# theo2021/OnDA

Hardware: AMD Instinct MI355X
Metric: adaptation-step images/sec (fwd+bwd+proto) 512x1024 bs=4 (higher is better)
Workload: dtype f32 (f16x2 split emulation); 1 GPU; hybrid_switch adaptation step (step + update_ema), 1024x512, bs=4 per micro-batch, 1 micro-batch(es) per GPU and optimizer step, dynamic branch, DeepLabV2-ResNet50 ProDA head, random-init weights; global_batch=4, parallelism=dp1, branch=dynamic, micro_batches_per_gpu=1, inputs=resident in HBM

## Files before the change

include/onda_hip.h:

```cpp
#ifndef ONDA_HIP_H
#define ONDA_HIP_H

#include <stdint.h>

#ifdef __cplusplus
extern "C" {
#endif

typedef void* onda_stream_t;

#define ONDA_OK 0
#define ONDA_EINVAL (-1)
#define ONDA_EALIGN (-2)

typedef struct OndaConv {
  int B, Hi, Wi, Cin;
  int Ho, Wo, Cout;
  int kh, kw, stride, dil, pad;
  int ldx;
  int ldy;
  int ldr;
  int out_os;
  int Hf, Wf;
  int relu;
// ... 66 lines not shown
                        float* running_mean, float* running_var, int64_t* nbt, float momentum, const float* gamma,
                        const float* beta, const float* res_amax, int relu, float* xhat_amax, float* out_amax, int64_t split,
                        int tile_rows, int run_group, const float* y, int ldy, onda_stream_t s);
int onda_bn_apply_l2(const float* x, const float* mean, const float* invstd, const float* gamma, const float* beta,
                     const void* res, int64_t res_plane, const float* res_amax, void* out, int64_t out_plane,
                     const float* out_amax, int64_t M, int C, int relu, uint8_t* relu_mask, int64_t split, onda_stream_t s);
int onda_bn_train_l2(const float* x, const float* partials, int tiles, float eps, float* mean, float* invstd, float* running_mean,
                     float* running_var, int64_t* nbt, float momentum, const float* gamma, const float* beta, const void* res,
                     const float* res_amax, int relu, float* xhat_amax, void* out, float* out_amax, int64_t M, int C,
                     uint8_t* relu_mask, int64_t split, int tile_rows, int run_group, onda_stream_t s);
int64_t onda_bn_bwd_l2_ws(int64_t M, int C);
int onda_bn_bwd_l2(const float* dout, const void* out, int64_t out_plane, const float* x, const float* mean, const float* invstd,
                   const float* gamma, const float* xhat_amax, void* dx, int64_t dx_plane, float* dx_amax, float* dres, float* ws,
                   int64_t M, int C, int relu, const uint8_t* relu_mask, int64_t split, int fuse_sums, onda_stream_t s);

int onda_conv_wgrad_l2_variant(int Cout, int Cin);
int64_t onda_conv2d_wgrad_l2_table_stride(const OndaConv* c);
int onda_conv2d_wgrad_l2_table(const OndaConv* c, int32_t* table, onda_stream_t s);
int onda_conv2d_wgrad_l2(const void* xl, int64_t xplane, const float* xamax, const void* dyl, int64_t dyplane, const float* dyamax,
                         float* slabs, int lddy, int splitk, const OndaConv* c, onda_stream_t s);

int onda_conv2d_wgrad(const float* x, const float* dy, float* slabs, int lddy, int splitk,
                      const OndaConv* c, onda_stream_t s);
int onda_wgrad_reduce(const float* slabs, float* dw, int splitk, int Cout, int taps, int Cin,
                      int Cout_real, int Cin_real, int flat_k, int accumulate, onda_stream_t s);

int onda_pack_weight_fwd(const float* w_oihw, float* dst, int Cout, int Cin, int taps, int Cout_pad, int Kp,
                         onda_stream_t s);
int onda_pack_weight_dgrad(const float* w_oihw, float* dst, int Cout, int Cin, int taps, int Cout_pad,
                           onda_stream_t s);
// ... 160 lines not shown
```

onda_amd/_lib.py:

```python
import ctypes
import os
from ctypes import POINTER, Structure, c_char_p, c_float, c_int, c_int64, c_void_p

HERE = os.path.dirname(os.path.abspath(__file__))
LIB_PATH = os.environ.get("ONDA_LIB_PATH") or os.path.join(HERE, "libonda_hip.so")

P = c_void_p
I, L, F = c_int, c_int64, c_float


class OndaConv(Structure):
    _fields_ = [(n, c_int) for n in ("B Hi Wi Cin Ho Wo Cout kh kw stride dil pad ldx ldy ldr out_os Hf Wf relu").split()] + \
               [("run_if", c_void_p), ("stat_split", c_int64), ("plain_schedule", c_int), ("pix_table", c_void_p),
                ("pix_stride", c_int64)]


class OndaSwitchCfg(Structure):
    _fields_ = [("limit", c_int), ("level_kind", c_int), ("use_exp", c_int), ("pad_", c_int), ("exp_const", ctypes.c_double),
                ("one_minus_exp_const", ctypes.c_double), ("taps_total", ctypes.c_double), ("gray_lo", ctypes.c_double),
                ("gray_hi", ctypes.c_double), ("dev_threshold", ctypes.c_double)]


class OndaLimbOut(Structure):
    _fields_ = [("out", c_void_p), ("out_plane", c_int64), ("out_bound", c_void_p), ("out_amax", c_void_p), ("kb", c_void_p),
                ("xtrue", c_void_p), ("res", c_void_p), ("res_plane", c_int64), ("res_amax", c_void_p), ("res_true", c_void_p)]


class OndaSgdEntry(Structure):
    _fields_ = [("p", c_void_p), ("g", c_void_p), ("buf", c_void_p), ("n", c_int64), ("lr", c_float),
                ("times", c_int), ("fresh", c_int), ("first_block", c_int)]


class OndaSgdAnchorEntry(Structure):
    _fields_ = [("p", c_void_p), ("g", c_void_p), ("buf", c_void_p), ("anchor", c_void_p), ("n", c_int64), ("lr", c_float),
                ("times", c_int), ("fresh", c_int), ("first_block", c_int)]


class OndaSqdiffEntry(Structure):
    _fields_ = [("a", c_void_p), ("b", c_void_p), ("n", c_int64), ("first_block", c_int)]

# ... 35 lines not shown
    "onda_conv_l2_kernel_id": (I, [L, I, I, I]),
    "onda_conv_l2_tiles_m": (I, [L, I, I, I]),
    "onda_conv_l2_tiles_m_split": (I, [L, I, I, I, L, I, POINTER(c_int)]),
    "onda_conv_l2_live_fraction": (ctypes.c_double, [POINTER(OndaConv), I]),
    "onda_conv_wgrad_l2_live_fraction": (ctypes.c_double, [POINTER(OndaConv), I]),
    "onda_conv_wgrad_l2_variant": (I, [I, I]),
    "onda_conv2d_wgrad_l2_table_stride": (L, [POINTER(OndaConv)]),
    "onda_conv2d_wgrad_l2_table": (I, [POINTER(OndaConv), P, P]),
    "onda_conv2d_wgrad_l2": (I, [P, L, P, P, L, P, P, I, I, POINTER(OndaConv), P]),
    "onda_conv2d_fwd_l2": (I, [P, L, P, P, P, P, P, P, P, P, I, P, P, POINTER(OndaConv), P]),
    "onda_bn_finalize_l2": (I, [P, I, I, L, F, P, P, P, P, P, F, P, P, P, I, P, P, L, I, I, P, I, P]),
    "onda_bn_apply_l2": (I, [P, P, P, P, P, P, L, P, P, L, P, L, I, I, P, L, P]),
    "onda_bn_bwd_l2_ws": (L, [L, I]),
    "onda_bn_train_l2": (I, [P, P, I, F, P, P, P, P, P, F, P, P, P, P, I, P, P, P, L, I, P, L, I, I, P]),
    "onda_bn_bwd_l2": (I, [P, P, L, P, P, P, P, P, P, L, P, P, P, L, I, I, P, L, I, P]),
    "onda_conv2d_wgrad": (I, [P, P, P, I, I, POINTER(OndaConv), P]),
    "onda_wgrad_reduce": (I, [P, P, I, I, I, I, I, I, I, I, P]),
    "onda_pack_weight_fwd": (I, [P, P, I, I, I, I, I, P]),
    "onda_pack_weight_dgrad": (I, [P, P, I, I, I, I, P]),
    "onda_stem_im2col": (I, [P, P, I, I, I, I, I, I, P]),
    "onda_bn_finalize": (I, [P, I, I, L, F, P, P, P, P, P, F, P]),
    "onda_bn_stats": (I, [P, L, I, I, P, POINTER(c_int), P]),
    "onda_bn_apply": (I, [P, P, P, P, P, P, P, L, I, I, P, P]),
    "onda_bn_fold": (I, [P, P, P, P, F, P, P, I, P]),
    "onda_bn_bwd_ws": (L, [L, I]),
    "onda_bn_bwd": (I, [P, P, P, P, P, P, P, P, P, L, I, I, P, P]),
    "onda_gn_ws": (L, [I, L, I]),
    "onda_gn_fwd": (I, [P, I, P, P, P, P, I, P, P, P, I, L, I, I, F, I, P, P]),
    "onda_gn_bwd": (I, [P, I, P, I, P, I, P, P, P, P, P, P, P, P, I, L, I, I, I, P]),
    "onda_gn_site_ws": (L, [I, L, I]),
# ... 90 lines not shown
```

onda_amd/csrc/norm_l2.hip:

```cpp
#include "limbs.h"

namespace {

#define LD4(p) (*reinterpret_cast<const f32x4*>(p))

__device__ __forceinline__ void store_limb_lines(_Float16* o, u32x4 l1, u32x4 l2, bool whole) {
  if (!whole) {
    *reinterpret_cast<u32x4*>(o) = l1;
    *reinterpret_cast<u32x4*>(o + LIMB2_OFS) = l2;
    return;
  }
  const bool hi = (threadIdx.x & 4) != 0;
  const u32x4 send = hi ? l1 : l2;
  u32x4 recv;
#pragma unroll
  for (int j = 0; j < 4; ++j) recv[j] = (unsigned)__shfl_xor((int)send[j], 4, 64);
  const unsigned long long mine = reinterpret_cast<unsigned long long>(o);
  const unsigned long long partner = ((unsigned long long)(unsigned)__shfl_xor((int)(mine >> 32), 4, 64) << 32) |
                                     (unsigned)__shfl_xor((int)(unsigned)mine, 4, 64);
  _Float16* po = reinterpret_cast<_Float16*>(partner);
  _Float16* a1 = hi ? po + LIMB2_OFS : o;
  _Float16* a2 = hi ? o + LIMB2_OFS : po;
  *reinterpret_cast<u32x4*>(a1) = hi ? recv : l1;
  *reinterpret_cast<u32x4*>(a2) = hi ? l2 : recv;
// ... 110 lines not shown
  const float* partials;
  int tiles, C;
  double count;
  float eps;
  float *mean, *invstd, *rmean, *rvar;
  int64_t* nbt;
  float momentum;
  const float *gamma, *beta, *res_amax;
  int relu;
  float *xhat_amax, *out_amax;
  long long split;
  int bm, run_group;
  const float* y;
  int ldy;
};
__device__ __forceinline__ void bn_finalize_block(const BnFinalizeArgs& a, const int bx, const int g) {
  const float* __restrict__ partials = a.partials;
  const int tiles = a.tiles, C = a.C, relu = a.relu, bm = a.bm, run_group = a.run_group, ldy = a.ldy;
  double count = a.count;
  const float eps = a.eps, momentum = a.momentum;
  float *mean = a.mean, *invstd = a.invstd, *rmean = a.rmean, *rvar = a.rvar, *xhat_amax = a.xhat_amax, *out_amax = a.out_amax;
  int64_t* nbt = a.nbt;
  const float* __restrict__ gamma = a.gamma;
  const float* __restrict__ beta = a.beta;
  const float* __restrict__ res_amax = a.res_amax;
  const float* __restrict__ y = a.y;
  const long long split = a.split;
  if (bx == 0 && g == 0 && threadIdx.x == 0 && nbt) *nbt += 1;
  int row0 = 0, nrows = tiles;
  if (split > 0) {
    const int ts = (int)(split / bm);
    if (g == 0) nrows = ts; else row0 = ts, nrows = tiles - ts;
    count = g == 0 ? (double)split : count - (double)split;
  }
  const long long m_all = (long long)a.count;
  const int tiles_m = bm > 1 ? (int)((m_all + bm - 1) / bm) : tiles, extra = tiles - tiles_m;
  int sub1 = 0;
  bool known = y != nullptr && bm > 1 && extra >= 0;
  if (known && extra > 0) {
    const bool d15 = extra % 15 == 0 && extra / 15 <= tiles_m, d31 = bm == 256 && extra % 31 == 0 && extra / 31 <= tiles_m;
// ... 7 lines not shown
    float mn = 3.0e38f, mx = -3.0e38f;
    if (bx * 16 + c < C)
      for (long long r = (split > last0 ? split : last0) + lane; r < m_all; r += 16) {
        const float v = y[(size_t)r * ldy + bx * 16 + c];
        mn = fminf(mn, v);
        mx = fmaxf(mx, v);
      }
    lmn[lane][c] = mn;
    lmx[lane][c] = mx;
  }
  double sum[2];
  float ext[2];
  reduce_rows16<4, 2, true>(partials + (size_t)row0 * 4 * C, nrows, C, bx * 16, sum, ext, rescan ? nrows - sub1 : nrows,
                            rescan ? tiles_m - 1 - row0 : -1);
  const int ch = bx * 16 + threadIdx.x;
  float bound = 0.f;
  if (threadIdx.x < 16 && ch < C) {
    if (rescan) {
#pragma unroll
      for (int l = 0; l < 16; ++l) {
        ext[0] = fminf(ext[0], lmn[l][threadIdx.x]);
        ext[1] = fmaxf(ext[1], lmx[l][threadIdx.x]);
      }
    }
    if (split > 0 && split % bm != 0) {
      double c1 = 0.0, c2 = 0.0;
      float mn = 3.0e38f, mx = -3.0e38f;
      for (long long r = split - split % bm; r < split; ++r) {
        const float v = y[(size_t)r * ldy + ch];
        c1 += (double)v;
        c2 += (double)v * (double)v;
// ... 4 lines not shown
        sum[0] += c1;
        sum[1] += c2;
        ext[0] = fminf(ext[0], mn);
        ext[1] = fmaxf(ext[1], mx);
      } else {
        sum[0] -= c1;
        sum[1] -= c2;
      }
    }
    const double mu = sum[0] / count;
    double var = sum[1] / count - mu * mu;
    if (var < 0.0) var = 0.0;
    const float muf = (float)mu, is = (float)(1.0 / sqrt(var + (double)eps));
    const float lo = (ext[0] - muf) * is, hi = (ext[1] - muf) * is;
    const float gm = gamma[ch], b = beta[ch];
    const float f_lo = lo * gm + b, f_hi = hi * gm + b;
    bound = relu ? fmaxf(0.f, fmaxf(f_lo, f_hi)) : fmaxf(fabsf(f_lo), fabsf(f_hi));
    mean[g * C + ch] = muf;
    invstd[g * C + ch] = is;
    xhat_amax[g * C + ch] = fmaxf(fabsf(lo), fabsf(hi));
    if (rmean && (split <= 0 || g == run_group)) {
      const double unbiased = count > 1.0 ? var * count / (count - 1.0) : var;
      rmean[ch] = (1.f - momentum) * rmean[ch] + momentum * muf;
      rvar[ch] = (1.f - momentum) * rvar[ch] + momentum * (float)unbiased;
    }
  }
  if (res_amax != nullptr) bound += amax_read(res_amax);
  bound *= 1.0000005f;
  __shared__ float red[4];
  float m = wave_max(bound);
  if ((threadIdx.x & 63) == 0) red[threadIdx.x >> 6] = m;
  __syncthreads();
  if (threadIdx.x == 0) {
    m = fmaxf(fmaxf(red[0], red[1]), fmaxf(red[2], red[3]));
    if (m > 0.f)
      atomicMax(reinterpret_cast<unsigned*>(out_amax) + ((bx + 7 * g) & (ONDA_AMAX_SLOTS - 1)) * AMAX_STRIDE, __float_as_uint(m));
  }
}
__global__ __launch_bounds__(256) void bn_finalize_l2_kernel(const BnFinalizeArgs a) { bn_finalize_block(a, blockIdx.x, blockIdx.y); }

template <bool FUSED>
__global__ __launch_bounds__(256) void bn_apply_l2_kernel(const float* __restrict__ x, const float* mean, const float* invstd,
                                                          const float* __restrict__ gamma, const float* __restrict__ beta,
                                                          const _Float16* __restrict__ res, size_t res_plane,
                                                          const float* __restrict__ res_amax, _Float16* __restrict__ out,
                                                          size_t out_plane, const float* out_amax, size_t total8, int C, int relu,
                                                          unsigned char* __restrict__ mask, size_t group1_at, const BnFinalizeArgs fin,
                                                          int nfin) {
  if constexpr (FUSED) {
    const int nb = (C + 15) / 16;
    if ((int)blockIdx.x < nfin) {
      bn_finalize_block(fin, blockIdx.x % nb, blockIdx.x / nb);
      grid_publish(fin.out_amax);
    }
// ... 49 lines not shown
      ra2 = ld_stream(reinterpret_cast<const u32x4*>(res + lofs(e) + LIMB2_OFS));
      rb1 = ld_stream(reinterpret_cast<const u32x4*>(res + lofs(f)));
      rb2 = ld_stream(reinterpret_cast<const u32x4*>(res + lofs(f) + LIMB2_OFS));
    }
    const bool whole = __ballot(1) == ~0ull;
    one(e, a0, a1, ra1, ra2, whole);
    one(f, b0, b1, rb1, rb2, whole);
  }
  if (e < total8) {
    u32x4 r1 = {}, r2 = {};
    if (res) {
      r1 = *reinterpret_cast<const u32x4*>(res + lofs(e));
      r2 = *reinterpret_cast<const u32x4*>(res + lofs(e) + LIMB2_OFS);
    }
    one(e, LD4(x + e * 8), LD4(x + e * 8 + 4), r1, r2, __ballot(1) == ~0ull);
  }
}

struct ColPlan3 {
  int cx, ry, gridx, chunks;
  int64_t rows_per_chunk;
};
static inline ColPlan3 col_plan3(int64_t M, int C) {
  ColPlan3 p;
  const int c4 = C / 4;
  p.cx = 1;
  while (p.cx < c4 && p.cx < 64) p.cx <<= 1;
  p.ry = 256 / p.cx;
  p.gridx = (c4 + p.cx - 1) / p.cx;
  int64_t target = 2048 / p.gridx;
// ... 152 lines not shown
    f32x4 v[2];
#pragma unroll
    for (int h = 0; h < 2; ++h) {
      const size_t o = e * 8 + 4 * h;
      f32x4 g = LD4S(dout + o);
      if (relu) g = relu_mask4(out, mask, o, g, C);
      const f32x4 xh = (LD4S(x + o) - (second ? mu[1][h] : mu[0][h])) * (second ? is[1][h] : is[0][h]);
      v[h] = (second ? gi[1][h] : gi[0][h]) * (g - (second ? m1[1][h] : m1[0][h]) - xh * (second ? m2[1][h] : m2[0][h]));
    }
    u32x4 l1, l2;
    split8(v[0] * sd, v[1] * sd, l1, l2);
    store_limb_lines(dx + (size_t)((unsigned)e / (unsigned)c8) * 2 * (size_t)C + limb_at(0, col, C), l1, l2, __ballot(1) == ~0ull);
  }
}

__global__ __launch_bounds__(256) void chan_scale_limbs_kernel(const float* __restrict__ x, const float* __restrict__ gate,
                                                               _Float16* __restrict__ out, size_t plane,
                                                               const float* __restrict__ amax, int64_t HW, int C, size_t total8) {
  const int c8 = C / 8;
  const float so = scale_of(amax).s;
  for (size_t e = (size_t)blockIdx.x * blockDim.x + threadIdx.x; e < total8; e += (size_t)gridDim.x * blockDim.x) {
    const int col = (int)(e % c8) * 8;
    const size_t b = (e / c8) / HW;
    const f32x4 v0 = LD4S(x + e * 8) * LD4(gate + b * C + col), v1 = LD4S(x + e * 8 + 4) * LD4(gate + b * C + col + 4);
    u32x4 l1, l2;
    split8(v0 * so, v1 * so, l1, l2);
    _Float16* o = out + (size_t)((unsigned)e / (unsigned)c8) * 2 * (size_t)C + limb_at(0, col, C);
    st_stream(reinterpret_cast<u32x4*>(o), l1);
    st_stream(reinterpret_cast<u32x4*>(o + LIMB2_OFS), l2);
  }
// ... 115 lines not shown
  if (fuse_sums) {
    const int nfin = (C + 15) / 16 * groups;
    const unsigned grid = ew_grid(total8) > (unsigned)nfin ? ew_grid(total8) : (unsigned)nfin;
    hipLaunchKernelGGL(bn_bwd_apply_l2_kernel<true>, dim3(grid), dim3(256), 0, st, dout, static_cast<const _Float16*>(out),
                       (size_t)out_plane, x, mean, invstd, gamma, sums, static_cast<_Float16*>(dx), (size_t)dx_plane, dx_amax, total8, C,
                       (float)inv_m0, relu, relu_mask, (size_t)split * C / 8, (float)inv_m1, fin, nfin);
    return ONDA_LAUNCH_RESULT();
  }
  hipLaunchKernelGGL(bn_bwd_sums_l2_kernel, dim3((C + 15) / 16, groups), dim3(256), 0, st, fin);
  hipLaunchKernelGGL(bn_bwd_apply_l2_kernel<false>, dim3(ew_grid(total8)), dim3(256), 0, st, dout, static_cast<const _Float16*>(out),
                     (size_t)out_plane, x, mean, invstd, gamma, sums, static_cast<_Float16*>(dx), (size_t)dx_plane, dx_amax, total8,
                     C, (float)inv_m0, relu, relu_mask, (size_t)split * C / 8, (float)inv_m1, BnBwdSumsArgs{}, 0);
  return ONDA_LAUNCH_RESULT();
}

}
```

onda_amd/framework/model/deeplabv2.py:

```python
import os

import torch
import torch.nn as nn

from onda_amd import ops

affine_par = True


class HipConv2d(nn.Conv2d):

    def __init__(self, *args, **kwargs):
        super().__init__(*args, **kwargs)
        self._pack = ops._PackCache()

    def geom(self):
        return self.kernel_size[0], self.stride[0], self.dilation[0], self.padding[0]

    def forward(self, x, want_stats=False, cout_pad=None):
        k, stride, dil, pad = self.geom()
        return ops.Conv2dFn.apply(x, self.weight, self.bias, self._pack, stride, dil, pad, want_stats, cout_pad)


class HipBatchNorm2d(nn.BatchNorm2d):
# ... 19 lines not shown
        return new




def conv_bn(conv, bn, x, relu, residual=None):
    k, stride, dil, pad = conv.geom()
    if isinstance(bn, nn.GroupNorm):
        if residual is not None:
            raise NotImplementedError("onda_amd: GroupNorm with a residual add is not a site of the reference's models")
        y, stats = conv(x, want_stats=True)
        return ops.GNSiteFn.apply(y, stats, bn.weight, bn.bias, relu, bn.num_groups, bn.eps)
    if bn.training:
        limbs = ops.limb_mode(conv.out_channels)
        y, stats = conv(x, want_stats=4 if limbs else True)
        running = (bn.running_mean, bn.running_var, bn.num_batches_tracked) if bn.track_running_stats else None
        if bn.momentum is None:
            raise NotImplementedError("onda_amd: cumulative-average BatchNorm (momentum=None) is not on the hot path")
        fn = ops.BNTrainLimbFn if stats.shape[1] == 4 else ops.BNTrainFn
        return fn.apply(y, stats, bn.weight, bn.bias, residual, relu, running, bn.momentum)
    scale, shift = bn.folded()
    with torch.no_grad():
        wp = conv._pack.get_fwd(conv.weight)
        limb_out = None
        if ops.limb_mode(conv.out_channels) and ops._use_l2(wp, x.shape[3]):
            w = conv.weight
            key = (w.data_ptr(), w._version, id(scale), id(shift))
            hit = getattr(bn, "_bound_cache", None)
            if hit is None or hit[0] != key:
                hit = bn._bound_cache = (key, ops.fold_bounds(w, scale, shift), scale, shift)
            limb_out = hit[1]
        y, _, _ = ops.conv_forward(x, wp, k, stride, dil, pad, conv.out_channels, scale=scale, shift=shift, residual=residual,
                                   relu=relu, limb_out=limb_out)
    return y


class Bottleneck(nn.Module):
    expansion = 4

    def __init__(self, inplanes, planes, stride=1, dilation=1, downsample=None, norm_module=HipBatchNorm2d,
                 norm_grad=False):
        super().__init__()
        self.conv1 = HipConv2d(inplanes, planes, kernel_size=1, stride=stride, bias=False)
        self.bn1 = norm_module(planes, affine=affine_par)
        self.conv2 = HipConv2d(planes, planes, kernel_size=3, stride=1, padding=dilation, bias=False,
                               dilation=dilation)
        self.bn2 = norm_module(planes, affine=affine_par)
        self.conv3 = HipConv2d(planes, planes * 4, kernel_size=1, bias=False)
        self.bn3 = norm_module(planes * 4, affine=affine_par)
        if not norm_grad:
            for bn in (self.bn1, self.bn2, self.bn3):
                for p in bn.parameters():
                    p.requires_grad = False
        self.relu = nn.ReLU(inplace=True)
        self.downsample = downsample
        self.stride = stride

    def forward(self, x):
        ops.share_grad(x)
        y = conv_bn(self.conv1, self.bn1, x, True)
        y = conv_bn(self.conv2, self.bn2, y, True)
        if self.downsample is not None:
            residual = conv_bn(self.downsample[0], self.downsample[1], x, False)
        else:
            residual = x
        return conv_bn(self.conv3, self.bn3, y, True, residual)


class SEBlock(nn.Module):
    def __init__(self, inplanes, r=16):
        super().__init__()
        self.global_pool = nn.AdaptiveAvgPool2d((1, 1))
        self.se = nn.Sequential(nn.Linear(inplanes, inplanes // r), nn.ReLU(inplace=True),
                                nn.Linear(inplanes // r, inplanes), nn.Sigmoid())

    def forward(self, x):
        return ops.SEScaleFn.apply(x, self.se[0].weight, self.se[0].bias, self.se[2].weight, self.se[2].bias)
# ... 225 lines not shown
```

onda_amd/ops/__init__.py:

```python
import sys
import types

from . import _state, conv, core, disc, limbs, loss, norm, tables
from ._state import BN_EPS, GN_EPS, GN_GROUPS, HEAD_PAD, STEM_K

_FLAGS = ("CONV_MODE", "H2_PATH", "GRAD_READY", "PROFILE", "PREDICATE", "ROW_GROUPS", "LIMB_ONLY", "SHARE_GRADS", "FUSE_BN_FINALIZE",
          "GN_FUSED_STATS")

for _m in (core, limbs, tables, conv, norm, loss, disc):
    for _k, _v in vars(_m).items():
        if not _k.startswith("__") and _k not in _FLAGS and not isinstance(_v, types.ModuleType):
            globals()[_k] = _v
del _m, _k, _v


class _OpsModule(types.ModuleType):
    def __getattr__(self, name):
        if name in _FLAGS:
            return getattr(_state, name)
        raise AttributeError(f"module {self.__name__!r} has no attribute {name!r}")

    def __setattr__(self, name, value):
        if name in _FLAGS:
            setattr(_state, name, value)
# ... 6 lines not shown
```

onda_amd/ops/_state.py:

```python
import os

BN_EPS = 1e-5
GN_EPS = 1e-5
GN_GROUPS = 32
HEAD_PAD = 32
STEM_K = 160


CONV_MODE = os.environ.get("ONDA_CONV_MODE", "f16x2")

H2_PATH = "dma"

GRAD_READY = None

PROFILE = None



PREDICATE = None

ROW_GROUPS = 0

LIMB_ONLY = True

SHARE_GRADS = True

FUSE_BN_FINALIZE = os.environ.get("ONDA_FUSE_BN", "0") == "1"

GN_FUSED_STATS = os.environ.get("ONDA_GN_FUSED_STATS", "1") == "1"
```

onda_amd/ops/norm.py:

```python
import ctypes
import os
from ctypes import byref

import torch

from .. import _lib
from .._lib import OndaConv, OndaLimbOut, call, query
from . import _state
from ._state import BN_EPS, GN_EPS, GN_GROUPS, HEAD_PAD, STEM_K
from .core import _group_split, _p, _stream, as_nhwc, nhwc_ld
from .limbs import Limbs, _stat_tile_rows, amax_slot, is_limb_only, known_amax, limb_mode, limb_only, limbs_of, tag_amax
from .conv import _sink_give, _sink_of, colsum


class BNTrainFn(torch.autograd.Function):

    @staticmethod
    def _groups(B, H, W):
        split, M = _group_split(B, H, W), B * H * W
        return [(0, M)] if not split else [(0, split), (split, M - split)]

    @staticmethod
    def forward(ctx, y, stats, gamma, beta, residual, relu, running, momentum):
        B, H, W, C = y.shape
# ... 120 lines not shown
        need_res = ctx.has_res and ctx.needs_input_grad[4]
        dres = None
        if need_res:
            dres = torch.empty_like(y) if ctx.relu else dout
        ol = ctx.out_limbs
        call("onda_bn_bwd_l2", _p(dout), _p(ol.planes) if ol is not None else None, ol.plane if ol is not None else 0, _p(y),
             _p(mean), _p(invstd), _p(gamma), _p(xhat_amax), _p(planes), M * C, _p(dx_amax),
             _p(dres) if (need_res and ctx.relu) else None, _p(ws), M, C, int(ctx.relu), _p(ctx.relu_mask), ctx.split,
             int(_state.FUSE_BN_FINALIZE), _stream())
        dx = limb_only((B, H, W, C), dev, Limbs(planes, dx_amax, C, M * C))
        if need_res:
            dres = _sink_give(ctx.res_sink, dres, ctx.relu)
        return dx, None, None, None, dres, None, None, None


def fold_bounds(weight, scale, shift):
    with torch.no_grad():
        l1 = weight.detach().abs().sum(dim=(1, 2, 3))
        return torch.stack([(scale.abs() * l1).max(), shift.abs().max()]).float().contiguous()


def bn_eval_fold(gamma, beta, rm, rv):
    C = gamma.numel()
    scale = torch.empty(C, device=gamma.device, dtype=torch.float32)
    shift = torch.empty_like(scale)
    call("onda_bn_fold", _p(gamma), _p(beta), _p(rm), _p(rv), BN_EPS, _p(scale), _p(shift), C, _stream())
    return scale, shift


class MaxPoolFn(torch.autograd.Function):
# ... 173 lines not shown
```

Before: 43.40 images/s.

## Fuse downsample and main-branch BatchNorm pairs in bottleneck blocks

Adds paired BN kernels that finalize statistics for both the conv3 BN and the downsample BN in one launch. The forward pass normalizes both, adds them, applies ReLU and writes f16 limbs in a single pass. The backward pass reads dout once to compute both branches' reductions and dx. This removes the intermediate residual limb tensor and its separate write and read, and cuts kernel launches in the four downsample bottlenecks. In exchange it adds more code paths, and the amax bound for the sum is now computed from the two ranges rather than from the stored residual amax.

```diff
diff --git a/include/onda_hip.h b/include/onda_hip.h
--- a/include/onda_hip.h
+++ b/include/onda_hip.h
@@ -104,6 +104,24 @@
                    const float* gamma, const float* xhat_amax, void* dx, int64_t dx_plane, float* dx_amax, float* dres, float* ws,
                    int64_t M, int C, int relu, const uint8_t* relu_mask, int64_t split, int fuse_sums, onda_stream_t s);
 
+typedef struct OndaBnSide {
+  const float* x;
+  const float* partials;
+  int tiles, tile_rows;
+  float *mean, *invstd, *xhat_amax;
+  float *running_mean, *running_var;
+  int64_t* nbt;
+  float momentum;
+  const float *gamma, *beta;
+  void* dx;
+  float* dx_amax;
+} OndaBnSide;
+int onda_bn_pair_fwd_l2(const OndaBnSide* a, const OndaBnSide* b, float eps, int relu, void* out, float* out_amax, int64_t M, int C,
+                        uint8_t* relu_mask, int64_t split, int run_group, onda_stream_t s);
+int64_t onda_bn_pair_bwd_l2_ws(int64_t M, int C);
+int onda_bn_pair_bwd_l2(const float* dout, const uint8_t* relu_mask, const OndaBnSide* a, const OndaBnSide* b, float* ws, int64_t M,
+                        int C, int relu, int64_t split, onda_stream_t s);
+
 int onda_conv_wgrad_l2_variant(int Cout, int Cin);
 int64_t onda_conv2d_wgrad_l2_table_stride(const OndaConv* c);
 int onda_conv2d_wgrad_l2_table(const OndaConv* c, int32_t* table, onda_stream_t s);
diff --git a/onda_amd/_lib.py b/onda_amd/_lib.py
--- a/onda_amd/_lib.py
+++ b/onda_amd/_lib.py
@@ -24,6 +24,13 @@
 class OndaLimbOut(Structure):
     _fields_ = [("out", c_void_p), ("out_plane", c_int64), ("out_bound", c_void_p), ("out_amax", c_void_p), ("kb", c_void_p),
                 ("xtrue", c_void_p), ("res", c_void_p), ("res_plane", c_int64), ("res_amax", c_void_p), ("res_true", c_void_p)]
+
+
+class OndaBnSide(Structure):
+    _fields_ = [("x", c_void_p), ("partials", c_void_p), ("tiles", c_int), ("tile_rows", c_int), ("mean", c_void_p),
+                ("invstd", c_void_p), ("xhat_amax", c_void_p), ("running_mean", c_void_p), ("running_var", c_void_p),
+                ("nbt", c_void_p), ("momentum", c_float), ("gamma", c_void_p), ("beta", c_void_p), ("dx", c_void_p),
+                ("dx_amax", c_void_p)]
 
 
 class OndaSgdEntry(Structure):
@@ -89,6 +96,9 @@
     "onda_bn_bwd_l2_ws": (L, [L, I]),
     "onda_bn_train_l2": (I, [P, P, I, F, P, P, P, P, P, F, P, P, P, P, I, P, P, P, L, I, P, L, I, I, P]),
     "onda_bn_bwd_l2": (I, [P, P, L, P, P, P, P, P, P, L, P, P, P, L, I, I, P, L, I, P]),
+    "onda_bn_pair_fwd_l2": (I, [POINTER(OndaBnSide), POINTER(OndaBnSide), F, I, P, P, L, I, P, L, I, P]),
+    "onda_bn_pair_bwd_l2_ws": (L, [L, I]),
+    "onda_bn_pair_bwd_l2": (I, [P, P, POINTER(OndaBnSide), POINTER(OndaBnSide), P, L, I, I, L, P]),
     "onda_conv2d_wgrad": (I, [P, P, P, I, I, POINTER(OndaConv), P]),
     "onda_wgrad_reduce": (I, [P, P, I, I, I, I, I, I, I, I, P]),
     "onda_pack_weight_fwd": (I, [P, P, I, I, I, I, I, P]),
diff --git a/onda_amd/csrc/norm_l2.hip b/onda_amd/csrc/norm_l2.hip
--- a/onda_amd/csrc/norm_l2.hip
+++ b/onda_amd/csrc/norm_l2.hip
@@ -148,16 +148,15 @@
   const float* y;
   int ldy;
 };
-__device__ __forceinline__ void bn_finalize_block(const BnFinalizeArgs& a, const int bx, const int g) {
+__device__ __forceinline__ void bn_finalize_channel(const BnFinalizeArgs& a, const int bx, const int g, float& f_lo, float& f_hi) {
   const float* __restrict__ partials = a.partials;
-  const int tiles = a.tiles, C = a.C, relu = a.relu, bm = a.bm, run_group = a.run_group, ldy = a.ldy;
+  const int tiles = a.tiles, C = a.C, bm = a.bm, run_group = a.run_group, ldy = a.ldy;
   double count = a.count;
   const float eps = a.eps, momentum = a.momentum;
-  float *mean = a.mean, *invstd = a.invstd, *rmean = a.rmean, *rvar = a.rvar, *xhat_amax = a.xhat_amax, *out_amax = a.out_amax;
+  float *mean = a.mean, *invstd = a.invstd, *rmean = a.rmean, *rvar = a.rvar, *xhat_amax = a.xhat_amax;
   int64_t* nbt = a.nbt;
   const float* __restrict__ gamma = a.gamma;
   const float* __restrict__ beta = a.beta;
-  const float* __restrict__ res_amax = a.res_amax;
   const float* __restrict__ y = a.y;
   const long long split = a.split;
   if (bx == 0 && g == 0 && threadIdx.x == 0 && nbt) *nbt += 1;
@@ -195,7 +194,7 @@
   reduce_rows16<4, 2, true>(partials + (size_t)row0 * 4 * C, nrows, C, bx * 16, sum, ext, rescan ? nrows - sub1 : nrows,
                             rescan ? tiles_m - 1 - row0 : -1);
   const int ch = bx * 16 + threadIdx.x;
-  float bound = 0.f;
+  f_lo = f_hi = 0.f;
   if (threadIdx.x < 16 && ch < C) {
     if (rescan) {
 #pragma unroll
@@ -230,8 +229,8 @@
     const float muf = (float)mu, is = (float)(1.0 / sqrt(var + (double)eps));
     const float lo = (ext[0] - muf) * is, hi = (ext[1] - muf) * is;
     const float gm = gamma[ch], b = beta[ch];
-    const float f_lo = lo * gm + b, f_hi = hi * gm + b;
-    bound = relu ? fmaxf(0.f, fmaxf(f_lo, f_hi)) : fmaxf(fabsf(f_lo), fabsf(f_hi));
+    f_lo = lo * gm + b;
+    f_hi = hi * gm + b;
     mean[g * C + ch] = muf;
     invstd[g * C + ch] = is;
     xhat_amax[g * C + ch] = fmaxf(fabsf(lo), fabsf(hi));
@@ -241,8 +240,8 @@
       rvar[ch] = (1.f - momentum) * rvar[ch] + momentum * (float)unbiased;
     }
   }
-  if (res_amax != nullptr) bound += amax_read(res_amax);
-  bound *= 1.0000005f;
+}
+__device__ __forceinline__ void bn_bound_publish(float bound, float* out_amax, const int bx, const int g) {
   __shared__ float red[4];
   float m = wave_max(bound);
   if ((threadIdx.x & 63) == 0) red[threadIdx.x >> 6] = m;
@@ -253,7 +252,26 @@
       atomicMax(reinterpret_cast<unsigned*>(out_amax) + ((bx + 7 * g) & (ONDA_AMAX_SLOTS - 1)) * AMAX_STRIDE, __float_as_uint(m));
   }
 }
+__device__ __forceinline__ void bn_finalize_block(const BnFinalizeArgs& a, const int bx, const int g) {
+  float f_lo, f_hi;
+  bn_finalize_channel(a, bx, g, f_lo, f_hi);
+  float bound = a.relu ? fmaxf(0.f, fmaxf(f_lo, f_hi)) : fmaxf(fabsf(f_lo), fabsf(f_hi));
+  if (a.res_amax != nullptr) bound += amax_read(a.res_amax);
+  bound *= 1.0000005f;
+  bn_bound_publish(bound, a.out_amax, bx, g);
+}
 __global__ __launch_bounds__(256) void bn_finalize_l2_kernel(const BnFinalizeArgs a) { bn_finalize_block(a, blockIdx.x, blockIdx.y); }
+
+__global__ __launch_bounds__(256) void bn_finalize_pair_l2_kernel(const BnFinalizeArgs a, const BnFinalizeArgs b) {
+  float lo_a, hi_a, lo_b, hi_b;
+  bn_finalize_channel(a, blockIdx.x, blockIdx.y, lo_a, hi_a);
+  __syncthreads();
+  bn_finalize_channel(b, blockIdx.x, blockIdx.y, lo_b, hi_b);
+  const float lo = fminf(lo_a, hi_a) + fminf(lo_b, hi_b), hi = fmaxf(lo_a, hi_a) + fmaxf(lo_b, hi_b);
+  float bound = a.relu ? fmaxf(0.f, hi) : fmaxf(fabsf(lo), fabsf(hi));
+  bound += 1.0e-6f * (fmaxf(fabsf(lo_a), fabsf(hi_a)) + fmaxf(fabsf(lo_b), fabsf(hi_b)));
+  bn_bound_publish(bound, a.out_amax, blockIdx.x, blockIdx.y);
+}
 
 template <bool FUSED>
 __global__ __launch_bounds__(256) void bn_apply_l2_kernel(const float* __restrict__ x, const float* mean, const float* invstd,
@@ -333,6 +351,69 @@
       r2 = *reinterpret_cast<const u32x4*>(res + lofs(e) + LIMB2_OFS);
     }
     one(e, LD4(x + e * 8), LD4(x + e * 8 + 4), r1, r2, __ballot(1) == ~0ull);
+  }
+}
+
+struct BnPairSide {
+  const float *x, *mean, *invstd, *gamma, *beta;
+};
+__global__ __launch_bounds__(256) void bn_apply_pair_l2_kernel(const BnPairSide sa, const BnPairSide sb, _Float16* __restrict__ out,
+                                                               const float* __restrict__ out_amax, size_t total8, int C, int relu,
+                                                               unsigned char* __restrict__ mask, size_t group1_at) {
+  const float* __restrict__ xa = sa.x;
+  const float* __restrict__ xb = sb.x;
+  const int c8 = C / 8;
+  const float so = scale_of(out_amax).s;
+  const size_t e0 = (size_t)blockIdx.x * blockDim.x + threadIdx.x;
+  const int col = (int)(e0 % c8) * 8;
+  const size_t stride = (size_t)gridDim.x * blockDim.x;
+  const size_t lcol = limb_at(0, col, C);
+  auto lofs = [&](size_t e) { return (size_t)((unsigned)e / (unsigned)c8) * 2 * (size_t)C + lcol; };
+  const size_t cut = group1_at > 0 ? group1_at : total8;
+  size_t e = e0;
+#pragma unroll 1
+  for (int g = 0; g < 2; ++g) {
+    const size_t end = g == 0 ? cut : total8;
+    if (e >= end) continue;
+    const int go = g * C + col;
+    const f32x4 ga0 = LD4(sa.gamma + col), ga1 = LD4(sa.gamma + col + 4), gb0 = LD4(sb.gamma + col), gb1 = LD4(sb.gamma + col + 4);
+    const f32x4 sca0 = LD4(sa.invstd + go) * ga0, sca1 = LD4(sa.invstd + go + 4) * ga1;
+    const f32x4 scb0 = LD4(sb.invstd + go) * gb0, scb1 = LD4(sb.invstd + go + 4) * gb1;
+    const f32x4 mua0 = LD4(sa.mean + go), mua1 = LD4(sa.mean + go + 4), mub0 = LD4(sb.mean + go), mub1 = LD4(sb.mean + go + 4);
+    const f32x4 bea0 = LD4(sa.beta + col), bea1 = LD4(sa.beta + col + 4), beb0 = LD4(sb.beta + col), beb1 = LD4(sb.beta + col + 4);
+    auto one = [&](size_t i, f32x4 a0, f32x4 a1, f32x4 b0, f32x4 b1, bool whole) {
+      const f32x4 ta0 = (a0 - mua0) * sca0 + bea0, ta1 = (a1 - mua1) * sca1 + bea1;
+      const f32x4 tb0 = (b0 - mub0) * scb0 + beb0, tb1 = (b1 - mub1) * scb1 + beb1;
+      f32x4 v0 = ta0 + tb0, v1 = ta1 + tb1;
+      if (mask) {
+        unsigned bits = 0;
+#pragma unroll
+        for (int j = 0; j < 4; ++j) bits |= (v0[j] > 0.f ? 1u << j : 0u) | (v1[j] > 0.f ? 16u << j : 0u);
+        mask[i] = (unsigned char)bits;
+      }
+      if (relu) {
+#pragma unroll
+        for (int j = 0; j < 4; ++j) {
+          v0[j] = fmaxf(v0[j], 0.f);
+          v1[j] = fmaxf(v1[j], 0.f);
+        }
+      }
+      u32x4 l1, l2;
+      split8(v0 * so, v1 * so, l1, l2);
+      store_limb_lines(out + lofs(i), l1, l2, whole);
+    };
+    for (; e + stride < end; e += 2 * stride) {
+      const size_t f = e + stride;
+      const f32x4 a0 = LD4S(xa + e * 8), a1 = LD4S(xa + e * 8 + 4), b0 = LD4S(xb + e * 8), b1 = LD4S(xb + e * 8 + 4);
+      const f32x4 c0 = LD4S(xa + f * 8), c1 = LD4S(xa + f * 8 + 4), d0 = LD4S(xb + f * 8), d1 = LD4S(xb + f * 8 + 4);
+      const bool whole = __ballot(1) == ~0ull;
+      one(e, a0, a1, b0, b1, whole);
+      one(f, c0, c1, d0, d1, whole);
+    }
+    if (e < end) {
+      one(e, LD4S(xa + e * 8), LD4S(xa + e * 8 + 4), LD4S(xb + e * 8), LD4S(xb + e * 8 + 4), __ballot(1) == ~0ull);
+      e += stride;
+    }
   }
 }
 
@@ -515,6 +596,154 @@
   }
 }
 
+__global__ __launch_bounds__(256) void bn_bwd_reduce_pair_l2_kernel(const float* __restrict__ dout, const float* __restrict__ xa,
+                                                                    const float* __restrict__ xb, const float* __restrict__ mean_a,
+                                                                    const float* __restrict__ invstd_a, const float* __restrict__ mean_b,
+                                                                    const float* __restrict__ invstd_b, int64_t M, int C, int relu, int cx,
+                                                                    int64_t rows_per_chunk, float* __restrict__ partials,
+                                                                    const unsigned char* __restrict__ mask, int64_t split, int chunks0) {
+  __shared__ f32x4 red[4][256];
+  const int t = threadIdx.x;
+  const int ry_n = 256 / cx;
+  const int tx = t % cx, ty = t / cx;
+  const int col = (blockIdx.x * cx + tx) * 4;
+  const int chunk = blockIdx.y;
+  const bool second = split > 0 && chunk >= chunks0;
+  const int64_t r0 = second ? split + (int64_t)(chunk - chunks0) * rows_per_chunk : (int64_t)chunk * rows_per_chunk;
+  const int64_t r1 = min(split > 0 && !second ? split : M, r0 + rows_per_chunk);
+  f32x4 s1 = {0.f, 0.f, 0.f, 0.f}, s2 = {0.f, 0.f, 0.f, 0.f}, s3 = {0.f, 0.f, 0.f, 0.f}, s4 = {0.f, 0.f, 0.f, 0.f};
+  if (col < C) {
+    const int gofs = second ? C : 0;
+    const f32x4 mua = LD4(mean_a + gofs + col), isa = LD4(invstd_a + gofs + col);
+    const f32x4 mub = LD4(mean_b + gofs + col), isb = LD4(invstd_b + gofs + col);
+    for (int64_t r = r0 + ty; r < r1; r += ry_n) {
+      const size_t o = (size_t)r * C + col;
+      f32x4 g = LD4(dout + o);
+      const f32x4 va = LD4(xa + o), vb = LD4(xb + o);
+      if (relu) g = relu_mask4(nullptr, mask, o, g, C);
+      s1 += g;
+      s2 += g * ((va - mua) * isa);
+      s3 += g * ((vb - mub) * isb);
+#pragma unroll
+      for (int j = 0; j < 4; ++j) s4[j] = fmaxf(s4[j], fabsf(g[j]));
+    }
+  }
+  red[0][t] = s1;
+  red[1][t] = s2;
+  red[2][t] = s3;
+  red[3][t] = s4;
+  __syncthreads();
+  if (ty == 0 && col < C) {
+    for (int y = 1; y < ry_n; ++y) {
+      s1 += red[0][y * cx + tx];
+      s2 += red[1][y * cx + tx];
+      s3 += red[2][y * cx + tx];
+      const f32x4 o4 = red[3][y * cx + tx];
+#pragma unroll
+      for (int j = 0; j < 4; ++j) s4[j] = fmaxf(s4[j], o4[j]);
+    }
+    float* dst = partials + ((size_t)chunk * 4) * C + col;
+    *reinterpret_cast<f32x4*>(dst) = s1;
+    *reinterpret_cast<f32x4*>(dst + C) = s2;
+    *reinterpret_cast<f32x4*>(dst + 2 * C) = s3;
+    *reinterpret_cast<f32x4*>(dst + 3 * C) = s4;
+  }
+}
+
+struct BnBwdSumsSide {
+  const float *gamma, *invstd, *xhat_amax;
+  float* dx_amax;
+};
+struct BnBwdSumsPairArgs {
+  const float* partials;
+  int chunks, C;
+  double inv_m0, inv_m1;
+  BnBwdSumsSide a, b;
+  float* sums;
+  int chunks0, groups;
+};
+__global__ __launch_bounds__(256) void bn_bwd_sums_pair_l2_kernel(const BnBwdSumsPairArgs p) {
+  const int C = p.C, bx = blockIdx.x, g = blockIdx.y;
+  const int row0 = g == 0 ? 0 : p.chunks0, nrows = p.groups == 1 ? p.chunks : (g == 0 ? p.chunks0 : p.chunks - p.chunks0);
+  const double inv_m = g == 0 ? p.inv_m0 : p.inv_m1;
+  double sum[3];
+  float ext[1];
+  reduce_rows16<4, 3, false>(p.partials + (size_t)row0 * 4 * C, nrows, C, bx * 16, sum, ext, nrows);
+  const int ch = bx * 16 + threadIdx.x;
+  float bound_a = 0.f, bound_b = 0.f;
+  if (threadIdx.x < 16 && ch < C) {
+#pragma unroll
+    for (int v = 0; v < 3; ++v) p.sums[(g * 3 + v) * C + ch] = (float)sum[v];
+    const float gmax = ext[0], m1 = (float)(fabs(sum[0]) * inv_m);
+    bound_a = fabsf(p.a.gamma[ch] * p.a.invstd[g * C + ch]) * (gmax + m1 + p.a.xhat_amax[g * C + ch] * (float)(fabs(sum[1]) * inv_m));
+    bound_b = fabsf(p.b.gamma[ch] * p.b.invstd[g * C + ch]) * (gmax + m1 + p.b.xhat_amax[g * C + ch] * (float)(fabs(sum[2]) * inv_m));
+  }
+  bn_bound_publish(bound_a * 1.000001f, p.a.dx_amax, bx, g);
+  __syncthreads();
+  bn_bound_publish(bound_b * 1.000001f, p.b.dx_amax, bx, g);
+}
+
+struct BnBwdPairSide {
+  const float *x, *mean, *invstd, *gamma;
+  _Float16* dx;
+  const float* dx_amax;
+};
+__global__ __launch_bounds__(256) void bn_bwd_apply_pair_l2_kernel(const float* __restrict__ dout, const BnBwdPairSide sa,
+                                                                   const BnBwdPairSide sb, const float* __restrict__ sums, size_t total8,
+                                                                   int C, float inv_m0, float inv_m1, int relu,
+                                                                   const unsigned char* __restrict__ mask, size_t group1_at) {
+  const float* __restrict__ xa = sa.x;
+  const float* __restrict__ xb = sb.x;
+  _Float16* __restrict__ dxa = sa.dx;
+  _Float16* __restrict__ dxb = sb.dx;
+  const int c8 = C / 8;
+  const float sda = scale_of(sa.dx_amax).s, sdb = scale_of(sb.dx_amax).s;
+  const size_t e0 = (size_t)blockIdx.x * blockDim.x + threadIdx.x;
+  const int col = (int)(e0 % c8) * 8;
+  const size_t stride = (size_t)gridDim.x * blockDim.x;
+  const size_t lcol = limb_at(0, col, C);
+  const size_t cut = group1_at > 0 ? group1_at : total8;
+  size_t e = e0;
+#pragma unroll 1
+  for (int g = 0; g < 2; ++g) {
+    const size_t end = g == 0 ? cut : total8;
+    if (e >= end) continue;
+    const float im = g == 0 ? inv_m0 : inv_m1;
+    f32x4 m1[2], mua[2], gia[2], m2a[2], mub[2], gib[2], m2b[2];
+#pragma unroll
+    for (int h = 0; h < 2; ++h) {
+      const int cc = col + 4 * h, go = g * C + cc;
+      const f32x4 isa = LD4(sa.invstd + go), isb = LD4(sb.invstd + go);
+      m1[h] = LD4(sums + (size_t)(g * 3) * C + cc) * im;
+      mua[h] = LD4(sa.mean + go);
+      gia[h] = LD4(sa.gamma + cc) * isa;
+      m2a[h] = isa * (LD4(sums + (size_t)(g * 3 + 1) * C + cc) * im);
+      mub[h] = LD4(sb.mean + go);
+      gib[h] = LD4(sb.gamma + cc) * isb;
+      m2b[h] = isb * (LD4(sums + (size_t)(g * 3 + 2) * C + cc) * im);
+    }
+    for (; e < end; e += stride) {
+      f32x4 va[2], vb[2];
+#pragma unroll
+      for (int h = 0; h < 2; ++h) {
+        const size_t o = e * 8 + 4 * h;
+        f32x4 gr = LD4S(dout + o);
+        const f32x4 pa = LD4S(xa + o), pb = LD4S(xb + o);
+        if (relu) gr = relu_mask4(nullptr, mask, o, gr, C);
+        va[h] = gia[h] * (gr - m1[h] - (pa - mua[h]) * m2a[h]);
+        vb[h] = gib[h] * (gr - m1[h] - (pb - mub[h]) * m2b[h]);
+      }
+      const bool whole = __ballot(1) == ~0ull;
+      const size_t lo = (size_t)((unsigned)e / (unsigned)c8) * 2 * (size_t)C + lcol;
+      u32x4 l1, l2;
+      split8(va[0] * sda, va[1] * sda, l1, l2);
+      store_limb_lines(dxa + lo, l1, l2, whole);
+      split8(vb[0] * sdb, vb[1] * sdb, l1, l2);
+      store_limb_lines(dxb + lo, l1, l2, whole);
+    }
+  }
+}
+
 __global__ __launch_bounds__(256) void chan_scale_limbs_kernel(const float* __restrict__ x, const float* __restrict__ gate,
                                                                _Float16* __restrict__ out, size_t plane,
                                                                const float* __restrict__ amax, int64_t HW, int C, size_t total8) {
@@ -660,4 +889,65 @@
   return ONDA_LAUNCH_RESULT();
 }
 
-}
+static bool pair_side_ok(const OndaBnSide* s, bool backward) {
+  if (!s || !s->x || !s->mean || !s->invstd || !s->xhat_amax || !s->gamma) return false;
+  return backward ? s->dx && s->dx_amax : s->partials && s->beta && s->tiles >= 1;
+}
+
+int onda_bn_pair_fwd_l2(const OndaBnSide* a, const OndaBnSide* b, float eps, int relu, void* out, float* out_amax, int64_t M, int C,
+                        uint8_t* relu_mask, int64_t split, int run_group, onda_stream_t s) {
+  ONDA_REQUIRE(pair_side_ok(a, false) && pair_side_ok(b, false) && out && out_amax && M >= 1 && C >= 32 && C % 32 == 0);
+  ONDA_REQUIRE(256 % (C / 8) == 0);
+  ONDA_REQUIRE(split >= 0 && split < M);
+  ONDA_REQUIRE(split == 0 || (a->tile_rows > 0 && b->tile_rows > 0 && split / a->tile_rows < a->tiles && split / b->tile_rows < b->tiles));
+  if (!ONDA_ALIGNED16(a->x) || !ONDA_ALIGNED16(b->x) || !ONDA_ALIGNED16(out) || !ONDA_ALIGNED16(a->partials) || !ONDA_ALIGNED16(b->partials))
+    return ONDA_EALIGN;
+  hipStream_t st = ONDA_STREAM(s);
+  const BnFinalizeArgs fa = finalize_args(a->partials, a->tiles, C, M, eps, a->mean, a->invstd, a->running_mean, a->running_var, a->nbt,
+                                          a->momentum, a->gamma, a->beta, nullptr, relu, a->xhat_amax, out_amax, split, a->tile_rows,
+                                          run_group, a->x, C);
+  const BnFinalizeArgs fb = finalize_args(b->partials, b->tiles, C, M, eps, b->mean, b->invstd, b->running_mean, b->running_var, b->nbt,
+                                          b->momentum, b->gamma, b->beta, nullptr, relu, b->xhat_amax, out_amax, split, b->tile_rows,
+                                          run_group, b->x, C);
+  hipLaunchKernelGGL(bn_finalize_pair_l2_kernel, dim3((C + 15) / 16, split > 0 ? 2 : 1), dim3(256), 0, st, fa, fb);
+  const size_t total8 = (size_t)M * C / 8;
+  hipLaunchKernelGGL(bn_apply_pair_l2_kernel, dim3(ew_grid(total8)), dim3(256), 0, st,
+                     BnPairSide{a->x, a->mean, a->invstd, a->gamma, a->beta}, BnPairSide{b->x, b->mean, b->invstd, b->gamma, b->beta},
+                     static_cast<_Float16*>(out), out_amax, total8, C, relu, relu_mask, (size_t)split * C / 8);
+  return ONDA_LAUNCH_RESULT();
+}
+
+int64_t onda_bn_pair_bwd_l2_ws(int64_t M, int C) {
+  const ColPlan3 p = col_plan3(M, C);
+  return (int64_t)(p.chunks + 1) * 4 * C + 6 * C;
+}
+
+int onda_bn_pair_bwd_l2(const float* dout, const uint8_t* relu_mask, const OndaBnSide* a, const OndaBnSide* b, float* ws, int64_t M,
+                        int C, int relu, int64_t split, onda_stream_t s) {
+  ONDA_REQUIRE(dout && pair_side_ok(a, true) && pair_side_ok(b, true) && ws && M >= 1 && C >= 32 && C % 32 == 0 && (!relu || relu_mask));
+  ONDA_REQUIRE(256 % (C / 8) == 0);
+  ONDA_REQUIRE(split >= 0 && split < M);
+  if (!ONDA_ALIGNED16(dout) || !ONDA_ALIGNED16(a->x) || !ONDA_ALIGNED16(b->x) || !ONDA_ALIGNED16(a->dx) || !ONDA_ALIGNED16(b->dx) ||
+      !ONDA_ALIGNED16(ws))
+    return ONDA_EALIGN;
+  const ColPlan3 p = col_plan3(M, C);
+  int chunks0, chunks;
+  bwd_chunks(p, M, split, chunks0, chunks);
+  float* sums = ws + (size_t)(p.chunks + 1) * 4 * C;
+  hipStream_t st = ONDA_STREAM(s);
+  hipLaunchKernelGGL(bn_bwd_reduce_pair_l2_kernel, dim3(p.gridx, chunks), dim3(256), 0, st, dout, a->x, b->x, a->mean, a->invstd, b->mean,
+                     b->invstd, M, C, relu, p.cx, p.rows_per_chunk, ws, relu_mask, split, chunks0);
+  const double inv_m0 = 1.0 / (double)(split > 0 ? split : M), inv_m1 = 1.0 / (double)(M - split);
+  const int groups = split > 0 ? 2 : 1;
+  hipLaunchKernelGGL(bn_bwd_sums_pair_l2_kernel, dim3((C + 15) / 16, groups), dim3(256), 0, st,
+                     BnBwdSumsPairArgs{ws, chunks, C, inv_m0, inv_m1, BnBwdSumsSide{a->gamma, a->invstd, a->xhat_amax, a->dx_amax},
+                                       BnBwdSumsSide{b->gamma, b->invstd, b->xhat_amax, b->dx_amax}, sums, chunks0, groups});
+  const size_t total8 = (size_t)M * C / 8;
+  hipLaunchKernelGGL(bn_bwd_apply_pair_l2_kernel, dim3(ew_grid(total8)), dim3(256), 0, st, dout,
+                     BnBwdPairSide{a->x, a->mean, a->invstd, a->gamma, static_cast<_Float16*>(a->dx), a->dx_amax},
+                     BnBwdPairSide{b->x, b->mean, b->invstd, b->gamma, static_cast<_Float16*>(b->dx), b->dx_amax}, sums, total8, C,
+                     (float)inv_m0, (float)inv_m1, relu, relu_mask, (size_t)split * C / 8);
+  return ONDA_LAUNCH_RESULT();
+}
+
+}
diff --git a/onda_amd/framework/model/deeplabv2.py b/onda_amd/framework/model/deeplabv2.py
--- a/onda_amd/framework/model/deeplabv2.py
+++ b/onda_amd/framework/model/deeplabv2.py
@@ -57,11 +57,8 @@
     if bn.training:
         limbs = ops.limb_mode(conv.out_channels)
         y, stats = conv(x, want_stats=4 if limbs else True)
-        running = (bn.running_mean, bn.running_var, bn.num_batches_tracked) if bn.track_running_stats else None
-        if bn.momentum is None:
-            raise NotImplementedError("onda_amd: cumulative-average BatchNorm (momentum=None) is not on the hot path")
         fn = ops.BNTrainLimbFn if stats.shape[1] == 4 else ops.BNTrainFn
-        return fn.apply(y, stats, bn.weight, bn.bias, residual, relu, running, bn.momentum)
+        return fn.apply(y, stats, bn.weight, bn.bias, residual, relu, _running(bn), bn.momentum)
     scale, shift = bn.folded()
     with torch.no_grad():
         wp = conv._pack.get_fwd(conv.weight)
@@ -76,6 +73,28 @@
         y, _, _ = ops.conv_forward(x, wp, k, stride, dil, pad, conv.out_channels, scale=scale, shift=shift, residual=residual,
                                    relu=relu, limb_out=limb_out)
     return y
+
+
+def _running(bn):
+    if bn.momentum is None:
+        raise NotImplementedError("onda_amd: cumulative-average BatchNorm (momentum=None) is not on the hot path")
+    return (bn.running_mean, bn.running_var, bn.num_batches_tracked) if bn.track_running_stats else None
+
+
+def pair_route(conv_a, bn_a, conv_b, bn_b):
+    return (ops.BN_PAIR and all(isinstance(bn, HipBatchNorm2d) and bn.training for bn in (bn_a, bn_b))
+            and conv_a.out_channels == conv_b.out_channels and ops.limb_mode(conv_a.out_channels))
+
+
+def conv_bn_pair(conv_a, bn_a, x_a, conv_b, bn_b, x_b, relu):
+    y_b, stats_b = conv_b(x_b, want_stats=4)
+    y_a, stats_a = conv_a(x_a, want_stats=4)
+    if ops.bn_pair_ok(y_a, stats_a, y_b, stats_b):
+        return ops.BNPairLimbFn.apply(y_a, stats_a, bn_a.weight, bn_a.bias, _running(bn_a), bn_a.momentum,
+                                      y_b, stats_b, bn_b.weight, bn_b.bias, _running(bn_b), bn_b.momentum, relu)
+    fns = [ops.BNTrainLimbFn if s.shape[1] == 4 else ops.BNTrainFn for s in (stats_a, stats_b)]
+    residual = fns[1].apply(y_b, stats_b, bn_b.weight, bn_b.bias, None, False, _running(bn_b), bn_b.momentum)
+    return fns[0].apply(y_a, stats_a, bn_a.weight, bn_a.bias, residual, relu, _running(bn_a), bn_a.momentum)
 
 
 class Bottleneck(nn.Module):
@@ -104,6 +123,8 @@
         y = conv_bn(self.conv1, self.bn1, x, True)
         y = conv_bn(self.conv2, self.bn2, y, True)
         if self.downsample is not None:
+            if pair_route(self.conv3, self.bn3, self.downsample[0], self.downsample[1]):
+                return conv_bn_pair(self.conv3, self.bn3, y, self.downsample[0], self.downsample[1], x, True)
             residual = conv_bn(self.downsample[0], self.downsample[1], x, False)
         else:
             residual = x
diff --git a/onda_amd/ops/__init__.py b/onda_amd/ops/__init__.py
--- a/onda_amd/ops/__init__.py
+++ b/onda_amd/ops/__init__.py
@@ -5,7 +5,7 @@
 from ._state import BN_EPS, GN_EPS, GN_GROUPS, HEAD_PAD, STEM_K
 
 _FLAGS = ("CONV_MODE", "H2_PATH", "GRAD_READY", "PROFILE", "PREDICATE", "ROW_GROUPS", "LIMB_ONLY", "SHARE_GRADS", "FUSE_BN_FINALIZE",
-          "GN_FUSED_STATS")
+          "GN_FUSED_STATS", "BN_PAIR")
 
 for _m in (core, limbs, tables, conv, norm, loss, disc):
     for _k, _v in vars(_m).items():
diff --git a/onda_amd/ops/_state.py b/onda_amd/ops/_state.py
--- a/onda_amd/ops/_state.py
+++ b/onda_amd/ops/_state.py
@@ -27,4 +27,6 @@
 
 FUSE_BN_FINALIZE = os.environ.get("ONDA_FUSE_BN", "0") == "1"
 
+BN_PAIR = os.environ.get("ONDA_BN_PAIR", "1") != "0"
+
 GN_FUSED_STATS = os.environ.get("ONDA_GN_FUSED_STATS", "1") == "1"
diff --git a/onda_amd/ops/norm.py b/onda_amd/ops/norm.py
--- a/onda_amd/ops/norm.py
+++ b/onda_amd/ops/norm.py
@@ -5,7 +5,7 @@
 import torch
 
 from .. import _lib
-from .._lib import OndaConv, OndaLimbOut, call, query
+from .._lib import OndaBnSide, OndaConv, OndaLimbOut, call, query
 from . import _state
 from ._state import BN_EPS, GN_EPS, GN_GROUPS, HEAD_PAD, STEM_K
 from .core import _group_split, _p, _stream, as_nhwc, nhwc_ld
@@ -158,6 +158,65 @@
         return dx, None, None, None, dres, None, None, None
 
 
+def bn_pair_ok(y_a, stats_a, y_b, stats_b):
+    return (stats_a is not None and stats_b is not None and stats_a.dim() == 3 and stats_b.dim() == 3
+            and stats_a.shape[1] == 4 and stats_b.shape[1] == 4 and y_a.dim() == 4 and y_a.shape == y_b.shape
+            and y_a.is_contiguous() and y_b.is_contiguous() and 256 % max(y_a.shape[3] // 8, 1) == 0)
+
+
+def _bn_side(y, stats, tile_rows, mean, invstd, xhat_amax, running, momentum, gamma, beta=None, dx=None, dx_amax=None):
+    rm, rv, nbt = running if running is not None else (None, None, None)
+    return OndaBnSide(_p(y), _p(stats), stats.shape[0] if stats is not None else 0, tile_rows, _p(mean), _p(invstd), _p(xhat_amax),
+                      _p(rm), _p(rv), _p(nbt), float(momentum), _p(gamma), _p(beta), _p(dx), _p(dx_amax))
+
+
+class BNPairLimbFn(torch.autograd.Function):
+
+    @staticmethod
+    def forward(ctx, y_a, stats_a, gamma_a, beta_a, running_a, momentum_a, y_b, stats_b, gamma_b, beta_b, running_b, momentum_b, relu):
+        B, H, W, C = y_a.shape
+        M = B * H * W
+        dev = y_a.device
+        if not bn_pair_ok(y_a, stats_a, y_b, stats_b):
+            raise RuntimeError("onda_amd: a BatchNorm pair needs two dense [B,H,W,C] conv outputs of one shape with four stat rows")
+        split = _group_split(B, H, W)
+        stat = [torch.empty((2 if split else 1) * C, device=dev, dtype=torch.float32) for _ in range(6)]
+        out_amax = amax_slot(dev)
+        rows = [_stat_tile_rows(s) if split else getattr(s, "_onda_tile_rows", 0) for s in (stats_a, stats_b)]
+        planes = torch.empty(2, M, C, device=dev, dtype=torch.float16)
+        mask = torch.empty(M * C // 8, device=dev, dtype=torch.uint8) if relu and any(ctx.needs_input_grad) else None
+        sa = _bn_side(y_a, stats_a, rows[0], stat[0], stat[1], stat[2], running_a, momentum_a, gamma_a, beta_a)
+        sb = _bn_side(y_b, stats_b, rows[1], stat[3], stat[4], stat[5], running_b, momentum_b, gamma_b, beta_b)
+        call("onda_bn_pair_fwd_l2", byref(sa), byref(sb), BN_EPS, int(relu), _p(planes), _p(out_amax), M, C, _p(mask), split, 1, _stream())
+        for running in (running_a, running_b):
+            if running is not None:
+                for t in running:
+                    torch.autograd.graph.increment_version(t)
+        ctx.split, ctx.relu, ctx.relu_mask = split, relu, mask
+        ctx.save_for_backward(y_a, y_b, gamma_a, gamma_b, *stat)
+        return limb_only((B, H, W, C), dev, Limbs(planes, out_amax, C, M * C))
+
+    @staticmethod
+    def backward(ctx, dout):
+        y_a, y_b, gamma_a, gamma_b, *stat = ctx.saved_tensors
+        B, H, W, C = y_a.shape
+        M = B * H * W
+        dev = y_a.device
+        if is_limb_only(dout):
+            raise RuntimeError("onda_amd: the gradient of a BatchNorm output must be an fp32 tensor")
+        if ctx.relu and ctx.relu_mask is None:
+            raise RuntimeError("onda_amd: a BatchNorm pair that ran without gradients has no ReLU mask to run backward with")
+        dout = dout.contiguous()
+        ws = torch.empty(query("onda_bn_pair_bwd_l2_ws", M, C), device=dev, dtype=torch.float32)
+        dx = [torch.empty(2, M, C, device=dev, dtype=torch.float16) for _ in range(2)]
+        amax = [amax_slot(dev) for _ in range(2)]
+        sa = _bn_side(y_a, None, 0, stat[0], stat[1], stat[2], None, 0.0, gamma_a, None, dx[0], amax[0])
+        sb = _bn_side(y_b, None, 0, stat[3], stat[4], stat[5], None, 0.0, gamma_b, None, dx[1], amax[1])
+        call("onda_bn_pair_bwd_l2", _p(dout), _p(ctx.relu_mask), byref(sa), byref(sb), _p(ws), M, C, int(ctx.relu), ctx.split, _stream())
+        da, db = (limb_only((B, H, W, C), dev, Limbs(dx[i], amax[i], C, M * C)) for i in range(2))
+        return da, None, None, None, None, None, db, None, None, None, None, None, None
+
+
 def fold_bounds(weight, scale, shift):
     with torch.no_grad():
         l1 = weight.detach().abs().sum(dim=(1, 2, 3))
```

Measured after the change: 44.01 images/s (median of 6 runs). +1.4%, better.
